# learningmatter-mit/surface-sampling

Measured on AMD Instinct MI355X. Metric: MC energy-evaluations/sec (SrTiO3(001) ~250-atom slabs, 3-model PaiNN ensemble E+F incl. neighbor list), higher is better.
Workload: dtype f32 via fp16x2-split MFMA (3 products), fp32 accumulate; neighbor decisions f64; 1 GPU; SrTiO3(001) PaiNN x3, 256 batched independent chains per GPU (BASELINE configs[3]), 248-272 atoms/chain; chains_per_gpu=256, atoms_per_gpu=66503, edges_per_gpu=2747786, slots_per_gpu=2836316, models=3, streams_per_gpu=2, parallelism=one GPU, no collective

## Files before the change

surface-sampling_amd/csrc/api_painn.hip:

```cpp
#include <cmath>

#include "vssr_internal.h"

namespace vssr {

static void transpose(const float *src, int rows, int cols, float *dst) {
    for (int r = 0; r < rows; ++r)
        for (int c = 0; c < cols; ++c) dst[(size_t)c * rows + r] = src[(size_t)r * cols + c];
}

static int upload_weights(vssr_handle *h, const vssr_painn_config *cfg) {
    const int M = cfg->n_models, L = cfg->num_conv, R = cfg->n_rbf, H = cfg->readout_hidden, NE = cfg->n_embed;
    const size_t per_layer = (size_t)F * F + F + (size_t)F3 * F + F3 + (size_t)F3 * R + F3 + 2 * (size_t)F * F +
                             (size_t)F * 2 * F + F + (size_t)F3 * F + F3;
    const size_t blob_len = (size_t)NE * F + L * per_layer + (size_t)H * F + H + H + 1;
    if (cfg->weights_len != blob_len)
        return set_err(h, VSSR_E_BADARG, "weights_len %llu does not match the layout (%zu floats)",
                       (unsigned long long)cfg->weights_len, blob_len);
    const size_t t_per_layer = (size_t)F * F + (size_t)F * F3 + 2 * (size_t)F * F + (size_t)2 * F * F + (size_t)F * F3;
    const size_t img_len = blob_len + L * t_per_layer + (size_t)F * H;
    std::vector<float> img(img_len * M);
    std::vector<ModelW> table(M);
    if (h->weights.ensure(img.size() * sizeof(float)))
        return set_err(h, VSSR_E_NOMEM, "weights: out of device memory");
// ... 107 lines not shown
            const float *b2 = hb + o; o += F3;
            const float *Wd = hb + o; o += (size_t)F3 * R;
            const float *bd = hb + o;
            l0_build_tables(hb, W1, b1, W2, b2, Wd, bd, NE, A.data() + per_model * m, At.data() + per_model * m);
        }
        const size_t pk = l0_packed_dwords(NE);
        std::vector<unsigned> A16(pk * M), At16(pk * M);
        for (int m = 0; m < M; ++m) l0_pack_tables(A.data() + per_model * m, NE, A16.data() + pk * m, At16.data() + pk * m);
        if (h->d_l0A.ensure(A16.size() * sizeof(unsigned)) || h->d_l0At.ensure(At16.size() * sizeof(unsigned)))
            return set_err(h, VSSR_E_NOMEM, "layer-0 tables");
        VSSR_HIP(h, hipMemcpy(h->d_l0A.p, A16.data(), A16.size() * sizeof(unsigned), hipMemcpyHostToDevice));
        VSSR_HIP(h, hipMemcpy(h->d_l0At.p, At16.data(), At16.size() * sizeof(unsigned), hipMemcpyHostToDevice));
    }
    if (h->model_table.ensure(sizeof(ModelW) * M)) return set_err(h, VSSR_E_NOMEM, "model table");
    VSSR_HIP(h, hipMemcpy(h->model_table.p, table.data(), sizeof(ModelW) * M, hipMemcpyHostToDevice));
    return VSSR_OK;
}

static void read_env_knobs(vssr_handle *h) {
    if (const char *e = getenv("VSSR_PAINN_PATH")) h->painn_general = h->painn_general || strcmp(e, "general") == 0;
    if (const char *e = getenv("VSSR_EDGE_IMPL")) h->edge_impl = (strcmp(e, "gather") == 0) ? 0 : 1;
    if (const char *e = getenv("VSSR_L0_FACTORISE")) h->l0_enabled = atoi(e);
    if (h->painn_general) h->l0_enabled = 0;
    if (const char *e = getenv("VSSR_UPD_SAVE")) h->upd_save = atoi(e);
    if (const char *e = getenv("VSSR_DEBUG_KEEP")) h->debug_keep = atoi(e);
    if (const char *e = getenv("VSSR_EDGE_FS16_MAX")) h->fs16_max_atoms = atoi(e);
    if (const char *e = getenv("VSSR_EDGE_FS8_MAX")) h->fs8_max_atoms = atoi(e);
    if (const char *e = getenv("VSSR_EDGE_BWD_MPASS")) h->bwd_multi_pass = atoi(e);
    if (const char *e = getenv("VSSR_EDGE_SUB_CHUNK")) { const int c = atoi(e); if (c >= 8) { h->sub_chunk_fwd = c; h->sub_chunk_bwd = c; } }
    if (const char *e = getenv("VSSR_EDGE_FWD_2PASS")) { const int w = atoi(e); h->fwd_two_pass = (w == 8 || w == 16) ? w : w ? 16 : 0; }
    if (const char *e = getenv("VSSR_EDGE_FWD_GRID")) h->edge_fwd_grid = max(atoi(e), 0);
}

}

using namespace vssr;

extern "C" {

int vssr_create(const vssr_painn_config *cfg, vssr_handle **out) {
    if (!cfg || !out) return set_err(nullptr, VSSR_E_BADARG, "null argument");
    *out = nullptr;
    if (cfg->struct_size != sizeof(vssr_painn_config))
        return set_err(nullptr, VSSR_E_BADARG, "vssr_painn_config size mismatch (%u vs %zu)", cfg->struct_size,
                       sizeof(vssr_painn_config));
    if (cfg->feat_dim < 16 || cfg->feat_dim > 256 || cfg->feat_dim % 16 != 0 || cfg->n_rbf < 1 || cfg->n_rbf > 32)
// ... 39 lines not shown
```

surface-sampling_amd/csrc/painn.hip:

```cpp
#include "vssr_internal.h"

namespace vssr {

constexpr int T = NODE_TILE;
constexpr int RB = 21;
constexpr int ECHUNK = 16;
constexpr float PI_F = 3.14159265358979323846f;

__device__ inline float sigmoidf_(float x) { return 1.f / (1.f + expf(-x)); }
__device__ inline float swishf_(float x) { return x * sigmoidf_(x); }
__device__ inline float dswishf_(float x) {
    float sg = sigmoidf_(x);
    return sg * fmaf(x, 1.f - sg, 1.f);
}

__global__ void __launch_bounds__(128) k_embed(int N, const int *__restrict__ Z, const ModelW *__restrict__ MW,
                                               float *__restrict__ s0, float *__restrict__ v0) {
    int i = blockIdx.x, m = blockIdx.y, f = threadIdx.x;
    const ModelW &W = MW[m];
    size_t a = (size_t)m * N + i;
    s0[a * F + f] = W.embed[(size_t)Z[i] * F + f];
    v0[(a * 3 + 0) * F + f] = 0.f;
    v0[(a * 3 + 1) * F + f] = 0.f;
    v0[(a * 3 + 2) * F + f] = 0.f;
// ... 556 lines not shown
        for (int c = 0; c < EDGE_MFMA_BCLASSES; o += h->n_bclass[c], ++c) bcls_list[c] = h->d_class_list.as<int>() + o;
    }
    const int n_gather = h->n_class[EDGE_CLASS_GATHER];
    const bool keep = h->upd_save && (want & VSSR_WANT_FORCES) && readout_mfma_supported(H);
    auto save_of = [&](int l) -> void * { return keep ? (char *)h->d_upd_save.p + update_save_bytes(N, M) * (size_t)l : nullptr; };
    h->l0_used = l0_fact;
    const bool fuse_last = readout_mfma_supported(H) && (want & VSSR_WANT_FORCES) && !keep;
    auto update_fwd = [&](int l) {
        const bool last = l + 1 == L;
        if (last && fuse_last && !h->debug_keep) return;
        P.begin(KC_UPDATE_FWD, st);
        launch_update_fwd_mfma(st, N, M, l, av, MW, sv.s_msg[l], sv.v_msg[l], sv.s_in[l + 1],
                               (!last || h->debug_keep) ? sv.v_in[l + 1] : nullptr, !last ? sv.phi[l + 1] : nullptr, save_of(l));
        P.end(st);
    };

    if (!l0_fact) {
        P.begin(KC_EMBED, st);
        hipLaunchKernelGGL(k_embed, g_atom, blk, 0, st, N, Z, MW, sv.s_in[0], sv.v_in[0]);
        P.end(st);
    }
    for (int l = 0; l < L; ++l) {
        if (l == 0 && l0_fact) {
            P.begin(KC_L0_FWD, st);
            rc = l0_run_forward(h, G, sv.s_msg[0], sv.v_msg[0]);
            if (rc) return rc;
            P.end(st);
            update_fwd(l);
            continue;
        }
        if (l == 0) {
            P.begin(KC_MSG_MLP, st);
            launch_msg_mlp_mfma(st, N, M, l, av, MW, sv.s_in[l], sv.phi[l]);
            P.end(st);
        }
        P.begin(KC_EDGE_FWD, st);
        if (l == 0)
            hipLaunchKernelGGL(k_edge_fwd<true>, g_atom, blk, 0, st, N, l, MW, G, counters, h->cutoff, h->excl_vol,
                               h->excl_sigma, h->excl_power, sv.s_in[l], sv.v_in[l], sv.phi[l], sv.s_msg[l],
                               sv.v_msg[l], -1);
        else {
            for (int cls = 0; cls < EDGE_MFMA_CLASSES; ++cls)
                launch_edge_fwd_mfma(st, cls, N, cls_list[cls], h->n_class[cls], M, l, h->max_class_atoms[cls], MW, G, counters,
                                     (int)(h->slot_cap - 1), sv.s_in[l], sv.v_in[l], sv.phi[l], sv.s_msg[l], sv.v_msg[l],
                                     (cls == EDGE_CLASS_FS4 && h->fwd_two_pass) ? h->d_bundle_sub.as<int4>() : (const int4 *)nullptr,
                                     h->fwd_two_pass, h->sub_chunk_fwd ? h->sub_chunk_fwd : sub_chunk_max(h->fwd_two_pass), h->edge_fwd_grid);
            if (n_gather)
                hipLaunchKernelGGL(k_edge_fwd<false>, g_atom, blk, 0, st, N, l, MW, G, counters, h->cutoff, h->excl_vol,
                                   h->excl_sigma, h->excl_power, sv.s_in[l], sv.v_in[l], sv.phi[l], sv.s_msg[l],
                                   sv.v_msg[l], (int)EDGE_BCLASS_GATHER);
        }
// ... 103 lines not shown
```

surface-sampling_amd/csrc/painn_l0.hip:

```cpp
#include "mfma16.h"

namespace vssr {

constexpr int KP = 24;
constexpr int TBLK = 4 * KP;

template <int NZ>
__global__ void __launch_bounds__(96)
k_l0_accum(GraphView G, const int *__restrict__ counters, float *__restrict__ T) {
    constexpr int nz = NZ;
    if (counters[2] || !G.act.atom(blockIdx.x)) return;
    const int i = blockIdx.x, comp = threadIdx.x / KP, kap = threadIdx.x % KP;
    float acc[NZ];
#pragma unroll
    for (int z = 0; z < NZ; ++z) acc[z] = 0.f;
    auto erec_c = [&](int idx) -> float4 {
#if defined(__HIP_DEVICE_COMPILE__)
        typedef const f32x4 __attribute__((address_space(4))) *cp;
        const f32x4 v = reinterpret_cast<cp>(reinterpret_cast<uintptr_t>(G.erec))[idx];
        return make_float4(v.x, v.y, v.z, v.w);
#else
        return G.erec[idx];
#endif
    };
    auto zslot_c = [&](int word) -> unsigned {
#if defined(__HIP_DEVICE_COMPILE__)
        typedef const unsigned __attribute__((address_space(4))) *cp;
// ... 6 lines not shown
    for (int e = e_begin; e < e_end; e += 4) {
        float4 er[4];
        float r[4];
        int zi[4];
        const unsigned zw = zslot_c(e >> 2);
#pragma unroll
        for (int u = 0; u < 4; ++u) {
            er[u] = erec_c(e + u);
            r[u] = G.rho[(size_t)(e + u) * KP + kap];
            zi[u] = (zw >> (8 * u)) & 255;
        }
#pragma unroll
        for (int u = 0; u < 4; ++u) {
            const float uu = comp == 0 ? 1.f : comp == 1 ? er[u].x : comp == 2 ? er[u].y : er[u].z;
            const float val = r[u] * uu;
#pragma unroll
            for (int z = 0; z < NZ; ++z) acc[z] += (z == zi[u]) ? val : 0.f;
        }
    }
#pragma unroll
    for (int z = 0; z < NZ; ++z) T[((size_t)i * nz + z) * TBLK + comp * KP + kap] = acc[z];
}

constexpr int L0_TILE_U4 = 1024;

__global__ void __launch_bounds__(NTHREADS)
k_l0_fwd16(int N, int M, int nz, ActiveView av, const int *__restrict__ counters, const int *__restrict__ Z,
           const int *__restrict__ zlist, const ModelW *__restrict__ MW, const uint4 *__restrict__ A16, int n_embed,
           const float *__restrict__ T, float *__restrict__ s_msg, float *__restrict__ v_msg) {
    extern __shared__ __attribute__((aligned(16))) _Float16 ldsh[];
    if (counters[2]) return;
    const int K = 32 * nz, a0 = blockIdx.x * TA;
    if (!av.tile(min(a0, N - 1), min(a0 + TA - 1, N - 1))) return;
    const Planes Ts = make_planes(ldsh, TA, K), Tv = make_planes(ldsh + plane_halves(TA, K), 3 * TA, K);
    const LaneGeo L;
    SatTrack sat;
    const int lane = threadIdx.x & 63, r = lane & 15, g = lane >> 4;
    for (int t = threadIdx.x; t < TA * nz * 4 * 8; t += NTHREADS) {
        const int k4 = t & 7, comp = (t >> 3) & 3, z = (t >> 5) % nz, a = t / (32 * nz);
        float4 val = make_float4(0.f, 0.f, 0.f, 0.f);
        if (4 * k4 < KP)
            val = *reinterpret_cast<const float4 *>(T + ((size_t)min(a0 + a, N - 1) * nz + z) * TBLK + comp * KP + 4 * k4);
        if (comp == 0) store_split4<SAT_ANY>(Ts, a, 32 * z + 4 * k4, val, sat);
        else store_split4<SAT_ANY>(Tv, (comp - 1) * TA + a, 32 * z + 4 * k4, val, sat);
    }
    sat.commit(av, a0, N);
    __syncthreads();
// ... 229 lines not shown
    for (int z = 0; z < n_embed; ++z)
        for (int sec = 0; sec < 2; ++sec) {
            std::fill(fk.begin(), fk.end(), 0.f);
            std::fill(kf.begin(), kf.end(), 0.f);
            for (int kap = 0; kap < KP; ++kap)
                for (int f = 0; f < F; ++f) {
                    const float v = A[(((size_t)z * 2 + sec) * KP + kap) * F + f];
                    fk[(size_t)f * 32 + kap] = v;
                    kf[(size_t)kap * F + f] = v;
                }
            const size_t o = ((size_t)z * 2 + sec) * L0_TILE_U4 * 4;
            pack_mfma_tiles16(fk.data(), F, 32, A16 + o);
            pack_mfma_tiles16(kf.data(), 32, F, At16 + o);
        }
}
size_t l0_packed_dwords(int n_embed) { return (size_t)n_embed * 2 * L0_TILE_U4 * 4; }

int l0_mfma_init(vssr_handle *h) {
    VSSR_HIP(h, hipFuncSetAttribute((const void *)k_l0_fwd16, hipFuncAttributeMaxDynamicSharedMemorySize, 160 * 1024));
    VSSR_HIP(h, hipFuncSetAttribute((const void *)k_l0_q16, hipFuncAttributeMaxDynamicSharedMemorySize, 160 * 1024));
    return VSSR_OK;
}

int l0_run_forward(vssr_handle *h, const GraphView &G, float *s_msg, float *v_msg) {
    const int N = h->n_atoms, M = h->n_models, nz = h->l0_nz;
    hipStream_t st = h->stream;
    if (h->d_l0T.ensure(sizeof(float) * (size_t)N * nz * TBLK) ||
        h->d_l0Q.ensure(sizeof(float) * (size_t)M * N * nz * TBLK))
        return set_err(h, VSSR_E_NOMEM, "layer-0 factorisation buffers: out of device memory");
    if (!h->l0T_by_geom) {
        const int *cnt = h->d_counters.as<int>();
        float *T = h->d_l0T.as<float>();
        switch (nz) {
            case 1: hipLaunchKernelGGL(k_l0_accum<1>, dim3(N), dim3(96), 0, st, G, cnt, T); break;
            case 2: hipLaunchKernelGGL(k_l0_accum<2>, dim3(N), dim3(96), 0, st, G, cnt, T); break;
            case 3: hipLaunchKernelGGL(k_l0_accum<3>, dim3(N), dim3(96), 0, st, G, cnt, T); break;
            case 4: hipLaunchKernelGGL(k_l0_accum<4>, dim3(N), dim3(96), 0, st, G, cnt, T); break;
            case 5: hipLaunchKernelGGL(k_l0_accum<5>, dim3(N), dim3(96), 0, st, G, cnt, T); break;
            case 6: hipLaunchKernelGGL(k_l0_accum<6>, dim3(N), dim3(96), 0, st, G, cnt, T); break;
            case 7: hipLaunchKernelGGL(k_l0_accum<7>, dim3(N), dim3(96), 0, st, G, cnt, T); break;
            default: hipLaunchKernelGGL(k_l0_accum<L0_MAX_SPECIES>, dim3(N), dim3(96), 0, st, G, cnt, T); break;
        }
    }
    const size_t lds_fwd = sizeof(_Float16) * (plane_halves(TA, 32 * nz) + plane_halves(3 * TA, 32 * nz));
    hipLaunchKernelGGL(k_l0_fwd16, dim3((N + TA - 1) / TA), dim3(NTHREADS), lds_fwd, st, N, M, nz, G.act, h->d_counters.as<int>(),
                       h->d_Z.as<int>(), h->d_zlist.as<int>(), h->model_table.as<ModelW>(), h->d_l0A.as<uint4>(), h->n_embed,
                       h->d_l0T.as<float>(), s_msg, v_msg);
    return VSSR_OK;
}

int l0_run_reverse(vssr_handle *h, const GraphView &G, int first_write, int fresh_mfma, const float *sbar_msg, const float *vbar_msg,
                   float4 *gbar) {
    const int N = h->n_atoms, M = h->n_models, nz = h->l0_nz;
    hipStream_t st = h->stream;
    const size_t lds_q = sizeof(_Float16) * (plane_halves(TA, F) + plane_halves(3 * TA, F));
    hipLaunchKernelGGL(k_l0_q16, dim3((N + TA - 1) / TA, M), dim3(NTHREADS), lds_q, st, N, nz, G.act, h->d_counters.as<int>(),
                       h->d_zlist.as<int>(), h->d_l0At.as<uint4>(), h->n_embed, sbar_msg, vbar_msg, h->d_l0Q.as<float>());
    if (sizeof(float) * 4 * M * nz * TBLK > 48 * 1024)
        VSSR_HIP(h, hipFuncSetAttribute((const void *)k_l0_bwd, hipFuncAttributeMaxDynamicSharedMemorySize, 160 * 1024));
    hipLaunchKernelGGL(k_l0_bwd, dim3((N + 3) / 4), dim3(256), sizeof(float) * 4 * M * nz * TBLK, st, N, M, nz, first_write, fresh_mfma,
                       h->excl_vol, h->cutoff, G, h->d_counters.as<int>(), h->d_l0Q.as<float>(), gbar, (long long)h->slot_cap);
    return VSSR_OK;
}

}
```

surface-sampling_amd/csrc/painn_node_mfma.hip:

```cpp
#include "mfma16.h"

#ifdef PHASE_TIMING
__device__ unsigned long long g_phase[64];
#define PH_INIT unsigned long long ph_t = wall_clock64();
#define PH_RESET ph_t = wall_clock64();
#define PH(k) { const unsigned long long ph_n = wall_clock64(); if (threadIdx.x == 0) atomicAdd(&g_phase[k], ph_n - ph_t); ph_t = wall_clock64(); }
extern "C" int vssr_debug_phases(unsigned long long *out, int reset) {
    if (hipMemcpyFromSymbol(out, HIP_SYMBOL(g_phase), sizeof(unsigned long long) * 64) != hipSuccess) return -1;
    if (reset) { unsigned long long z[64] = {}; if (hipMemcpyToSymbol(HIP_SYMBOL(g_phase), z, sizeof(z)) != hipSuccess) return -1; }
    return 0;
}
#else
#define PH_INIT
#define PH_RESET
#define PH(k)
#endif

namespace vssr {

template <int NRT, int NCT>
struct GemmShape {
    static constexpr int NT = NRT * NCT, NACC = NT >= 3 ? 1 : 2;
};
template <int NRT, int NCT, int NPRE>
// ... 395 lines not shown
        return v_msg + ((mN + a) * 3 + x) * F;
    }, sat);
}
template <int RT, class Sat>
__device__ __forceinline__ void load_update_s(_Float16 *ldsh, const float *__restrict__ s_msg, size_t mN, int a0, int N, Sat &sat) {
    constexpr int TA = 16 * RT;
    const Planes hs = make_planes(ldsh + UpdLds<RT>::OFF_HS, TA, 2 * F);
    load_rows_split<TA>(hs, 0, [&](int row) { return s_msg + (mN + min(a0 + row, N - 1)) * F; }, sat);
}

constexpr int CF_XS = plane_halves(3 * TA, F);
constexpr int CF_LDS_HALVES = CF_XS + plane_halves(TA, F);
static_assert(2 * plane_halves(TA, F) <= CF_XS, "|Vv| and swish planes overlay the v tile");
static_assert(4 * TA * FT * sizeof(float) <= CF_LDS_HALVES * sizeof(_Float16), "output tile overlays the planes");
#ifndef UPD_SAVE_LATE
#define UPD_SAVE_LATE 1
#endif
constexpr int UPD_SAVE_UV = 0, UPD_SAVE_H3 = 12, UPD_SAVE_GATE = 14, UPD_SAVE_REGS = 18;
__device__ __forceinline__ f32x4 &save_slot(f32x4 *save, int m, int k) {
    return save[(((size_t)m * gridDim.x + blockIdx.x) * UPD_SAVE_REGS + k) * NTHREADS + threadIdx.x];
}
size_t update_save_bytes(int N, int M) { return sizeof(f32x4) * (size_t)M * ((N + TA - 1) / TA) * UPD_SAVE_REGS * NTHREADS; }

template <int TAIL>
__global__ void __launch_bounds__(NTHREADS) __attribute__((amdgpu_waves_per_eu(2, 2)))
k_update_fwd_mfma(int N, int l, ActiveView av, const ModelW *__restrict__ MW, const float *__restrict__ s_msg,
                  const float *__restrict__ v_msg, float *__restrict__ s_out, float *__restrict__ v_out,
                  float *__restrict__ phi_next, f32x4 *__restrict__ save) {
    extern __shared__ __attribute__((aligned(16))) _Float16 ldsh[];
    constexpr bool NOV = TAIL == 2;
    const int m = blockIdx.y, a0 = blockIdx.x * TA;
    if (!av.tile(min(a0, N - 1), min(a0 + TA - 1, N - 1))) return;
    const LaneGeo L;
    SatTrack sat;
    const LayerW &W = MW[m].layer[l];
    const size_t mN = (size_t)m * N;
    const Planes vt = make_planes(ldsh, 3 * TA, F), xs = make_planes(ldsh + CF_XS, TA, F);
    const Planes nr = make_planes(ldsh, TA, F), as_ = make_planes(ldsh + plane_halves(TA, F), TA, F);
    constexpr int PF = 1;
    float4 keep_v[3 * TA * (F / 4) / NTHREADS], keep_s[TA * (F / 4) / NTHREADS];
    PH_INIT
    const uint4 *wUV[2] = {WTILE(U, L.w, F), WTILE(V, L.w, F)};
    const uint4 *wW3a[1] = {WTILE(W3, L.w, 2 * F)};
    const uint4 *wW3b[1] = {WTILE(W3, L.w, 2 * F) + (F / 32) * 2 * 64};
    const uint4 *wW4[3] = {WTILE(W4, L.w, F), WTILE(W4, NW + L.w, F), WTILE(W4, 2 * NW + L.w, F)};
    WPre<6, 2, 1> pUV;
    WPre<2, 1, 1> pW3a;
    rows_request<3 * TA>([&](int row) {
        int x = row / TA, a = min(a0 + (row % TA), N - 1);
        return v_msg + ((mN + a) * 3 + x) * F;
    }, keep_v);
    rows_request<TA>([&](int row) { return s_msg + (mN + min(a0 + row, N - 1)) * F; }, keep_s);
    __builtin_amdgcn_sched_barrier(0);
    gemm16_preload(wUV, pUV);
    gemm16_preload(wW3a, pW3a);
    rows_store_split<3 * TA>(vt, 0, keep_v, sat);
    rows_store_split<TA>(xs, 0, keep_s, sat);
    __syncthreads();
    PH(0)
    f32x4 uv[6][2];
    zero_acc(uv);
    gemm16<F, 6, 2, PF, 1>(vt, wUV, uv, &pUV);
    PH(1)
    f32x4 h3[2][1];
    zero_acc(h3);
    gemm16<F, 2, 1, PF, 1>(xs, wW3a, h3, &pW3a);
    WPre<2, 1, 2> pW3b;
    gemm16_preload(wW3b, pW3b);
    PH(2)
    __syncthreads();
    PH(3)
    f32x4 inner[2];
#pragma unroll
    for (int t = 0; t < 2; ++t) {
        f32x4 nv;
#pragma unroll
        for (int i = 0; i < 4; ++i) {
            float n2 = 0.f, in = 0.f;
#pragma unroll
            for (int x = 0; x < 3; ++x) {
// ... 65 lines not shown
        for (int j = 0; j < 6; ++j)
#pragma unroll
            for (int c = 0; c < 2; ++c) save_slot(save, m, UPD_SAVE_UV + 2 * j + c) = uv[j][c];
#pragma unroll
        for (int t = 0; t < 2; ++t) {
            save_slot(save, m, UPD_SAVE_H3 + t) = h3[t][0];
#pragma unroll
            for (int c = 0; c < 2; ++c) save_slot(save, m, UPD_SAVE_GATE + 2 * t + c) = gate[t][c];
        }
    };
#if UPD_SAVE_LATE == 0
    save_all();
#endif
    PH(7)
    __syncthreads();
    PH(8)
    float *T = reinterpret_cast<float *>(ldsh);
#pragma unroll
    for (int t = 0; t < 2; ++t) {
        const int row = L.row(t);
        f32x4 ds;
#pragma unroll
        for (int i = 0; i < 4; ++i) ds[i] = fmaf(gate[t][1][i], inner[t][i], gate[t][2][i]);
        *reinterpret_cast<f32x4 *>(T + row * FT + L.col0) = ds;
        if constexpr (!NOV) {
#pragma unroll
            for (int x = 0; x < 3; ++x) *reinterpret_cast<f32x4 *>(T + (TA * (1 + x) + row) * FT + L.col0) = gate[t][0] * uv[2 * x + t][0];
        }
    }
    __syncthreads();
    auto gofs = [&](int row, int col) -> size_t {
        const int q = row / TA, a = min(a0 + row % TA, N - 1);
        return q == 0 ? (mN + a) * F + col : ((mN + a) * 3 + (q - 1)) * F + col;
    };
    PH(9)
    const Planes xo = make_planes(ldsh + CF_LDS_HALVES, TA, F);
    auto put = [&](int row, int col, const float4 &d, const float4 &r) {
        const float4 o = make_float4(r.x + d.x, r.y + d.y, r.z + d.z, r.w + d.w);
        if (TAIL == 1 && row < TA) store_split4<SAT_COOP>(xo, row, col, o, sat);
        if (a0 + row % TA >= N) return;
        if (row >= TA && !v_out) return;
        *reinterpret_cast<float4 *>((row < TA ? s_out : v_out) + gofs(row, col)) = o;
    };
    {
        constexpr int NS = TA * (F / 4) / NTHREADS, NV = 3 * TA * (F / 4) / NTHREADS;
#pragma unroll
        for (int it = 0; it < (NOV ? NS : NS + NV); ++it) {
            const int idx = threadIdx.x + it * NTHREADS, row = idx >> 5, c4 = idx & 31;
            put(row, 4 * c4, *reinterpret_cast<const float4 *>(T + row * FT + 4 * c4), it < NS ? keep_s[it < NS ? it : 0] : keep_v[it < NS ? 0 : it - NS]);
        }
    }
    PH(10)
    if constexpr (TAIL == 1) {
        const LayerW &Wn = MW[m].layer[l + 1];
        const Planes hn = make_planes(ldsh, TA, F);
        __syncthreads();
        WPre<2, 3, 1> pW2n;
        {
            f32x4 acc[2][1];
            zero_acc(acc);
            const f32x4 b = gload4f(Wn.b1 + L.col0);
            __builtin_amdgcn_sched_barrier(0);
            gemm16<F, 2, 1, 1, 2>(xo, wW1n, acc, &pW1n);
            gemm16_preload(wW2n, pW2n);
#pragma unroll
            for (int t = 0; t < 2; ++t) {
                f32x4 hv = acc[t][0] + b;
#pragma unroll
                for (int i = 0; i < 4; ++i) hv[i] = swish(hv[i]);
                store_split4(hn, L.row(t), L.col0, hv, sat);
            }
        }
        __syncthreads();
        f32x4 acc[2][3];
        zero_acc(acc);
        f32x4 b2[3];
#pragma unroll
        for (int c = 0; c < 3; ++c) b2[c] = gload4f(Wn.b2 + c * F + L.col0);
        __builtin_amdgcn_sched_barrier(0);
        gemm16<F, 2, 3, 1, 1>(hn, wW2n, acc, &pW2n);
#pragma unroll
        for (int c = 0; c < 3; ++c) {
            const f32x4 b = b2[c];
#pragma unroll
            for (int t = 0; t < 2; ++t) {
                const int a = a0 + L.row(t);
                if (a < N) *reinterpret_cast<f32x4 *>(phi_next + (mN + a) * F3 + c * F + L.col0) = acc[t][c] + b;
            }
        }
        PH(11)
    }
#if UPD_SAVE_LATE
    save_all();
#endif
    sat.commit(av, a0, N);
}

constexpr int RH = 64;
template <int RT, bool WANT_SBAR, class Sat>
__device__ __forceinline__ void readout_head(const ModelW &W, const Planes &xs, const Planes &hp, float *red, const LaneGeo &L,
                                             int a0, int N, size_t mN, const float *__restrict__ e_excl,
                                             float *__restrict__ e_atom, f32x4 (&sb)[RT], Sat &sat) {
    constexpr int NCW = RH / 16;
    constexpr int TA = 16 * RT;
    const int lane = threadIdx.x & 63;
    if (L.w < NCW) {
        f32x4 acc[RT][1];
        zero_acc(acc);
        const uint4 *wp[1] = {W.qW5 + (size_t)L.w * 4 * F};
        const f32x4 b = gload4f(W.b5 + L.col0), w6 = gload4f(W.w6 + L.col0);
        __builtin_amdgcn_sched_barrier(0);
        gemm16<F, RT, 1>(xs, wp, acc);
#pragma unroll
        for (int t = 0; t < RT; ++t) {
            const f32x4 hval = acc[t][0] + b;
            f32x4 hb;
            float es = 0.f;
#pragma unroll
// ... 374 lines not shown
        case 1: return sizeof(_Float16) * (plane_halves(TA, F) + plane_halves(TA, F3));
        case 4: return sizeof(_Float16) * (plane_halves(TA, F) + plane_halves(TA, RH)) + sizeof(float) * (RH / 16) * TA;
        case 6: return 96 * 1024;
        default: return sizeof(_Float16) * UpdLds<2>::HALVES + sizeof(float) * 3 * TA * FT;
    }
}
static_assert(sizeof(_Float16) * plane_halves(16, RH) + sizeof(float) * (RH / 16) * 16 <= sizeof(float) * 3 * 16 * FT,
              "readout scratch fits the vbar region");

static_assert(sizeof(_Float16) * (CF_LDS_HALVES + plane_halves(TA, F)) <= 96 * 1024, "update fwd LDS request");

bool readout_mfma_supported(int hidden) { return hidden == RH; }

int node_mfma_init(vssr_handle *h) {
    VSSR_HIP(h, hipFuncSetAttribute((const void *)k_msg_mlp_mfma<2, 0>, hipFuncAttributeMaxDynamicSharedMemorySize, 96 * 1024));
    VSSR_HIP(h, hipFuncSetAttribute((const void *)k_msg_mlp_bwd_mfma, hipFuncAttributeMaxDynamicSharedMemorySize,
                                    (int)node_mfma_lds_bytes(1)));
    VSSR_HIP(h, hipFuncSetAttribute((const void *)k_update_fwd_mfma<0>, hipFuncAttributeMaxDynamicSharedMemorySize,
                                    (int)node_mfma_lds_bytes(6)));
    VSSR_HIP(h, hipFuncSetAttribute((const void *)k_update_fwd_mfma<1>, hipFuncAttributeMaxDynamicSharedMemorySize,
                                    (int)node_mfma_lds_bytes(6)));
    VSSR_HIP(h, hipFuncSetAttribute((const void *)k_update_fwd_mfma<2>, hipFuncAttributeMaxDynamicSharedMemorySize,
                                    (int)node_mfma_lds_bytes(6)));
#define SET_UPD(MODE)                                                                                                     \
    VSSR_HIP(h, hipFuncSetAttribute((const void *)k_update_bwd_mfma<MODE, 2>, hipFuncAttributeMaxDynamicSharedMemorySize, \
                                    (int)node_mfma_lds_bytes(3)));
    SET_UPD(0) SET_UPD(2) SET_UPD(3)
#undef SET_UPD
    VSSR_HIP(h, hipFuncSetAttribute((const void *)k_update_bwd_mfma<1, 2, true>, hipFuncAttributeMaxDynamicSharedMemorySize,
                                    (int)node_mfma_lds_bytes(3)));
    VSSR_HIP(h, hipFuncSetAttribute((const void *)k_update_bwd_mfma<2, 2, true>, hipFuncAttributeMaxDynamicSharedMemorySize,
                                    (int)node_mfma_lds_bytes(3)));
    VSSR_HIP(h, hipFuncSetAttribute((const void *)k_readout_mfma, hipFuncAttributeMaxDynamicSharedMemorySize,
                                    (int)node_mfma_lds_bytes(4)));
    return VSSR_OK;
}

void launch_msg_mlp_mfma(hipStream_t st, int N, int M, int l, const ActiveView &av, const ModelW *MW, const float *s_in,
                         float *phi) {
    hipLaunchKernelGGL((k_msg_mlp_mfma<2, 0>), dim3((N + TA - 1) / TA, M), dim3(NTHREADS), node_mfma_lds_bytes(0), st, N, l, av, MW,
                       s_in, phi);
}
void launch_msg_mlp_bwd_mfma(hipStream_t st, int N, int M, int l, const ActiveView &av, const ModelW *MW, const float *s_in,
                             const float *phibar, const float *sbar_msg, float *sbar_in) {
    hipLaunchKernelGGL(k_msg_mlp_bwd_mfma, dim3((N + TA - 1) / TA, M), dim3(NTHREADS), node_mfma_lds_bytes(1), st, N, l, av, MW,
                       s_in, phibar, sbar_msg, sbar_in);
}
void launch_update_fwd_mfma(hipStream_t st, int N, int M, int l, const ActiveView &av, const ModelW *MW, const float *s_msg,
                            const float *v_msg, float *s_out, float *v_out, float *phi_next, void *save) {
    f32x4 *sv = reinterpret_cast<f32x4 *>(save);
    if (phi_next)
        hipLaunchKernelGGL(k_update_fwd_mfma<1>, dim3((N + TA - 1) / TA, M), dim3(NTHREADS), node_mfma_lds_bytes(6), st, N, l,
                           av, MW, s_msg, v_msg, s_out, v_out, phi_next, sv);
    else if (!v_out && !sv)
        hipLaunchKernelGGL(k_update_fwd_mfma<2>, dim3((N + TA - 1) / TA, M), dim3(NTHREADS), node_mfma_lds_bytes(6), st, N, l,
                           av, MW, s_msg, v_msg, s_out, v_out, phi_next, sv);
    else
        hipLaunchKernelGGL(k_update_fwd_mfma<0>, dim3((N + TA - 1) / TA, M), dim3(NTHREADS), node_mfma_lds_bytes(6), st, N, l,
                           av, MW, s_msg, v_msg, s_out, v_out, phi_next, sv);
}
void launch_readout_mfma(hipStream_t st, int N, int M, const ActiveView &av, const ModelW *MW, const float *s,
                         const float *e_excl, float *e_atom) {
    hipLaunchKernelGGL(k_readout_mfma, dim3((N + TA - 1) / TA, M), dim3(NTHREADS), node_mfma_lds_bytes(4), st, N, av, MW, s,
                       e_excl, e_atom);
}
void launch_update_bwd_mfma(hipStream_t st, int N, int M, int l, int mode, int vbar_is_zero, const ActiveView &av, const ModelW *MW,
                            const float *s_msg, const float *v_msg, const float *sbar_src, const float *vbar,
                            const float *s_next, const float *phibar, const float *e_excl, float *e_atom,
                            float *sbar_msg, float *vbar_msg, float *s_last, const void *save) {
    const f32x4 *sv = reinterpret_cast<const f32x4 *>(save);
    if (mode == 1 || mode == 3) vbar_is_zero = 1;
#if defined(UPD_BWD_RT) && UPD_BWD_RT == 1
    if (!sv && mode == 2) {
        const dim3 grid1((N + 15) / 16, M), blk1(NTHREADS);
        const size_t lds1 = sizeof(_Float16) * UpdLds<1>::HALVES + sizeof(float) * 3 * 16 * FT;
        static bool once = [] {
            (void)hipFuncSetAttribute((const void *)k_update_bwd_mfma<2, 1, false>, hipFuncAttributeMaxDynamicSharedMemorySize, 80 * 1024);
            return true;
        }();
        (void)once;
        hipLaunchKernelGGL((k_update_bwd_mfma<2, 1, false>), grid1, blk1, lds1, st, N, l, vbar_is_zero, av, MW, s_msg, v_msg, sbar_src,
                           vbar, s_next, phibar, e_excl, e_atom, sbar_msg, vbar_msg, s_last, sv);
// ... 17 lines not shown
```

surface-sampling_amd/csrc/vssr_internal.h:

```cpp
#pragma once

#include <hip/hip_runtime.h>

#include <cstdint>
#include <cstdio>
#include <cstdlib>
#include <cstring>
#include <initializer_list>
#include <memory>
#include <string>
#include <type_traits>
#include <utility>
#include <vector>

#include "../../include/vssr_eval.h"

namespace vssr {

constexpr int F = 128;
constexpr int F3 = 3 * F;
constexpr int MAX_LAYERS = 4;
constexpr int MAX_MODELS = 8;
constexpr int RB_MAX = 24;
constexpr int NODE_TILE = 8;
// ... 340 lines not shown
    int cm_cap_per_atom = 0;
    int cg_driver = 0;
    int cg_last_driver = 0;
    bool cap_tight = false;
    vssr::DevBuf d_md_vel;
    vssr::DevBuf d_md_aux;
    bool md_vel_valid = false;
    int md_driver = 0;
    int md_last_driver = 0;
    vssr::DevBuf d_vib;
    vssr::DevBuf d_neb;
    vssr::DevBuf d_dimer;
    vssr::DevBuf d_npt;
    vssr::DevBuf d_cellrelax;
    uint32_t last_want = 0;
    int64_t slot_cap = 0;
    vssr::PinnedInts h_counters;

    vssr::DevBuf d_state;
    vssr::StateView sv;
    vssr::DevBuf d_gbar;
    vssr::DevBuf d_upd_save;
    vssr::DevBuf d_gpart;
    int debug_keep = 0;
    int upd_save = 0;
    vssr::DevBuf d_energy, d_energy_std, d_energy_models, d_forces, d_forces_std, d_e_atoms;
    vssr::DevBuf d_energy64;
    vssr::DevBuf d_pot_e, d_pot_ea, d_pot_f;
    vssr::DevBuf d_sat, d_sat_out;
    std::vector<unsigned> h_sat;
    bool h_sat_valid = false;
    vssr::DevBuf d_stress;

    int gmm_K = 0, gmm_D = 0, gmm_Dp = 0;
    double gmm_log2pi = 0.0;
    vssr::DevBuf d_gmm_P;
    vssr::DevBuf d_gmm_c;
    vssr::DevBuf d_gmm_kc;
    vssr::DevBuf d_gmm_mask;
    vssr::DevBuf d_gmm_x, d_gmm_lp, d_gmm_nll, d_gmm_sys, d_gmm_start;
    std::unique_ptr<vssr::GmmFit> fit;
    std::unique_ptr<vssr::Cluster> clu;
};

namespace vssr {

// ... 104 lines not shown
int chain_min_cg(vssr_handle *h, const vssr_cg_params *cp, const uint8_t *fixed_host, uint32_t want);
int node_mfma_init(vssr_handle *h);
void launch_msg_mlp_mfma(hipStream_t st, int N, int M, int l, const ActiveView &av, const ModelW *MW, const float *s_in,
                         float *phi);
void launch_msg_mlp_bwd_mfma(hipStream_t st, int N, int M, int l, const ActiveView &av, const ModelW *MW, const float *s_in,
                             const float *phibar, const float *sbar_msg, float *sbar_in);
void launch_update_fwd_mfma(hipStream_t st, int N, int M, int l, const ActiveView &av, const ModelW *MW, const float *s_msg,
                            const float *v_msg, float *s_out, float *v_out, float *phi_next, void *save);
size_t update_save_bytes(int N, int M);
bool readout_mfma_supported(int hidden);
void launch_readout_mfma(hipStream_t st, int N, int M, const ActiveView &av, const ModelW *MW, const float *s, const float *e_excl,
                         float *e_atom);
void launch_update_bwd_mfma(hipStream_t st, int N, int M, int l, int mode, int vbar_is_zero, const ActiveView &av, const ModelW *MW,
                            const float *s_msg, const float *v_msg, const float *sbar_src, const float *vbar,
                            const float *s_next, const float *phibar, const float *e_excl, float *e_atom,
                            float *sbar_msg, float *vbar_msg, float *s_last, const void *save);
void pack_mfma_tiles16(const float *Wsrc, int rows, int K, unsigned *dst );
void build_wd16(const float *Wd, const float *bd, unsigned *dst );
void l0_build_tables(const float *blob_embed, const float *W1, const float *b1, const float *W2, const float *b2,
                     const float *Wd, const float *bd, int n_embed, float *A, float *At);
void l0_pack_tables(const float *A, int n_embed, unsigned *A16, unsigned *At16);
size_t l0_packed_dwords(int n_embed);
int l0_mfma_init(vssr_handle *h);
int l0_run_forward(vssr_handle *h, const GraphView &G, float *s_msg, float *v_msg);
int l0_run_reverse(vssr_handle *h, const GraphView &G, int first_write, int fresh_mfma, const float *sbar_msg, const float *vbar_msg,
                   float4 *gbar);
int edge_mfma_init(vssr_handle *h);
enum { EDGE_CLASS_FS16 = 0, EDGE_CLASS_FS16M = 1, EDGE_CLASS_FS8 = 2, EDGE_CLASS_FS4 = 3, EDGE_CLASS_GATHER = 4, EDGE_CLASSES = 5,
       EDGE_MFMA_CLASSES = 4 };
enum { EDGE_BCLASS_FS16 = 0, EDGE_BCLASS_FS8 = 1, EDGE_BCLASS_FS4 = 2, EDGE_BCLASS_FS16P = 3, EDGE_BCLASS_GATHER = 4, EDGE_BCLASSES = 5,
       EDGE_MFMA_BCLASSES = 4 };
__host__ __device__ constexpr int edge_bclass_slices(int c) { return (c == EDGE_BCLASS_FS16 || c == EDGE_BCLASS_FS16P) ? 8 : c == EDGE_BCLASS_FS8 ? 16 : c == EDGE_BCLASS_FS4 ? 32 : 1; }
int edge_bclass_of(int n_atoms);
int edge_class_of(int n_atoms);
constexpr int SUB_MAX_PASSES = 4;
__host__ __device__ constexpr int sub_chunk_max(int width) { return width == 16 ? 400 : 784; }
__host__ __device__ constexpr int sub_chunk_max_bwd() { return 550; }
__host__ __device__ constexpr int sub_passes(int n_atoms, int chunk_max) { return (n_atoms + chunk_max - 1) / chunk_max; }
__host__ __device__ constexpr int sub_chunk(int n_atoms, int chunk_max) { return (n_atoms + sub_passes(n_atoms, chunk_max) - 1) / sub_passes(n_atoms, chunk_max); }
int edge_class_groups(int cls);
void launch_edge_bwd_mfma(hipStream_t st, int cls, int N, const int *list, int n_list, int M, int l, int max_atoms,
                          const ModelW *MW, const GraphView &G, const int *counters, int zero_slot,
                          const float *v_in, const float *phi, const float *sbar_msg, const float *vbar_msg,
                          float *phibar, float *vbar_in, float *gpart, long long slot_cap, int n_groups, int group_off,
                          const int4 *bundle_sub, int sub_chunk);
void launch_edge_fwd_mfma(hipStream_t st, int cls, int N, const int *list, int n_list, int M, int l, int max_atoms, const ModelW *MW,
                          const GraphView &G, const int *counters, int zero_slot, const float *s_in, const float *v_in,
// ... 5 lines not shown
```

Before: 25420 evaluations/s.

## Fuse layer-0 factorised message contraction into the first update kernel

When layer-0 factorisation is active and the number of species is at most four, the separate k_l0_fwd16 contraction kernel is skipped. The first update_fwd kernel now loads the per-atom T tables and packed A16 weights, computes the layer-0 messages with MFMA in its prologue, and adds them directly to the update residual. It still writes s_msg/v_msg for the backward pass. This removes one kernel launch and a global round trip of the message tensors. In exchange the fused kernel needs much more LDS (up to 160 KB), which may lower occupancy.

```diff
diff --git a/surface-sampling_amd/csrc/api_painn.hip b/surface-sampling_amd/csrc/api_painn.hip
--- a/surface-sampling_amd/csrc/api_painn.hip
+++ b/surface-sampling_amd/csrc/api_painn.hip
@@ -153,6 +153,7 @@
     if (const char *e = getenv("VSSR_EDGE_IMPL")) h->edge_impl = (strcmp(e, "gather") == 0) ? 0 : 1;
     if (const char *e = getenv("VSSR_L0_FACTORISE")) h->l0_enabled = atoi(e);
     if (h->painn_general) h->l0_enabled = 0;
+    if (const char *e = getenv("VSSR_L0_FUSE")) h->l0_fuse = atoi(e);
     if (const char *e = getenv("VSSR_UPD_SAVE")) h->upd_save = atoi(e);
     if (const char *e = getenv("VSSR_DEBUG_KEEP")) h->debug_keep = atoi(e);
     if (const char *e = getenv("VSSR_EDGE_FS16_MAX")) h->fs16_max_atoms = atoi(e);
diff --git a/surface-sampling_amd/csrc/painn.hip b/surface-sampling_amd/csrc/painn.hip
--- a/surface-sampling_amd/csrc/painn.hip
+++ b/surface-sampling_amd/csrc/painn.hip
@@ -602,11 +602,19 @@
     }
     for (int l = 0; l < L; ++l) {
         if (l == 0 && l0_fact) {
+            const bool l0_fuse = h->l0_fuse && h->l0T_by_geom && h->l0_nz <= L0_FUSE_MAX_SPECIES && L >= 2;
             P.begin(KC_L0_FWD, st);
-            rc = l0_run_forward(h, G, sv.s_msg[0], sv.v_msg[0]);
+            rc = l0_run_forward(h, G, sv.s_msg[0], sv.v_msg[0], l0_fuse);
             if (rc) return rc;
             P.end(st);
-            update_fwd(l);
+            if (!l0_fuse) {
+                update_fwd(l);
+                continue;
+            }
+            const L0FuseArgs f0{h->d_l0T.as<float>(), h->d_l0A.as<uint4>(), h->d_zlist.as<int>(), Z, counters, h->l0_nz, h->n_embed};
+            P.begin(KC_UPDATE_FWD, st);
+            launch_update_fwd_l0_mfma(st, N, M, av, MW, f0, sv.s_msg[0], sv.v_msg[0], sv.s_in[1], sv.v_in[1], sv.phi[1], save_of(0));
+            P.end(st);
             continue;
         }
         if (l == 0) {
diff --git a/surface-sampling_amd/csrc/painn_l0.hip b/surface-sampling_amd/csrc/painn_l0.hip
--- a/surface-sampling_amd/csrc/painn_l0.hip
+++ b/surface-sampling_amd/csrc/painn_l0.hip
@@ -2,7 +2,7 @@
 
 namespace vssr {
 
-constexpr int KP = 24;
+constexpr int KP = L0_KP;
 constexpr int TBLK = 4 * KP;
 
 template <int NZ>
@@ -55,7 +55,6 @@
     for (int z = 0; z < NZ; ++z) T[((size_t)i * nz + z) * TBLK + comp * KP + kap] = acc[z];
 }
 
-constexpr int L0_TILE_U4 = 1024;
 
 __global__ void __launch_bounds__(NTHREADS)
 k_l0_fwd16(int N, int M, int nz, ActiveView av, const int *__restrict__ counters, const int *__restrict__ Z,
@@ -331,7 +330,7 @@
     return VSSR_OK;
 }
 
-int l0_run_forward(vssr_handle *h, const GraphView &G, float *s_msg, float *v_msg) {
+int l0_run_forward(vssr_handle *h, const GraphView &G, float *s_msg, float *v_msg, bool fused) {
     const int N = h->n_atoms, M = h->n_models, nz = h->l0_nz;
     hipStream_t st = h->stream;
     if (h->d_l0T.ensure(sizeof(float) * (size_t)N * nz * TBLK) ||
@@ -351,6 +350,7 @@
             default: hipLaunchKernelGGL(k_l0_accum<L0_MAX_SPECIES>, dim3(N), dim3(96), 0, st, G, cnt, T); break;
         }
     }
+    if (fused) return VSSR_OK;
     const size_t lds_fwd = sizeof(_Float16) * (plane_halves(TA, 32 * nz) + plane_halves(3 * TA, 32 * nz));
     hipLaunchKernelGGL(k_l0_fwd16, dim3((N + TA - 1) / TA), dim3(NTHREADS), lds_fwd, st, N, M, nz, G.act, h->d_counters.as<int>(),
                        h->d_Z.as<int>(), h->d_zlist.as<int>(), h->model_table.as<ModelW>(), h->d_l0A.as<uint4>(), h->n_embed,
diff --git a/surface-sampling_amd/csrc/painn_node_mfma.hip b/surface-sampling_amd/csrc/painn_node_mfma.hip
--- a/surface-sampling_amd/csrc/painn_node_mfma.hip
+++ b/surface-sampling_amd/csrc/painn_node_mfma.hip
@@ -441,14 +441,17 @@
 }
 size_t update_save_bytes(int N, int M) { return sizeof(f32x4) * (size_t)M * ((N + TA - 1) / TA) * UPD_SAVE_REGS * NTHREADS; }
 
-template <int TAIL>
-__global__ void __launch_bounds__(NTHREADS) __attribute__((amdgpu_waves_per_eu(2, 2)))
-k_update_fwd_mfma(int N, int l, ActiveView av, const ModelW *__restrict__ MW, const float *__restrict__ s_msg,
-                  const float *__restrict__ v_msg, float *__restrict__ s_out, float *__restrict__ v_out,
-                  float *__restrict__ phi_next, f32x4 *__restrict__ save) {
-    extern __shared__ __attribute__((aligned(16))) _Float16 ldsh[];
+struct L0None {};
+template <int TAIL, bool L0F, class L0A>
+__device__ __forceinline__ void
+update_fwd_block(_Float16 *ldsh, int N, int l, const ActiveView &av, const ModelW *__restrict__ MW, const float *__restrict__ s_msg,
+                 const float *__restrict__ v_msg, float *__restrict__ s_out, float *__restrict__ v_out,
+                 float *__restrict__ phi_next, f32x4 *__restrict__ save, const L0A &f0, float *__restrict__ s_msg_w,
+                 float *__restrict__ v_msg_w) {
+    static_assert(!L0F || TAIL == 1, "the fused first block is the TAIL = 1 form");
     constexpr bool NOV = TAIL == 2;
     const int m = blockIdx.y, a0 = blockIdx.x * TA;
+    if constexpr (L0F) { if (f0.counters[2]) return; }
     if (!av.tile(min(a0, N - 1), min(a0 + TA - 1, N - 1))) return;
     const LaneGeo L;
     SatTrack sat;
@@ -457,7 +460,8 @@
     const Planes vt = make_planes(ldsh, 3 * TA, F), xs = make_planes(ldsh + CF_XS, TA, F);
     const Planes nr = make_planes(ldsh, TA, F), as_ = make_planes(ldsh + plane_halves(TA, F), TA, F);
     constexpr int PF = 1;
-    float4 keep_v[3 * TA * (F / 4) / NTHREADS], keep_s[TA * (F / 4) / NTHREADS];
+    float4 keep_v[L0F ? 1 : 3 * TA * (F / 4) / NTHREADS], keep_s[L0F ? 1 : TA * (F / 4) / NTHREADS];
+    f32x4 res[L0F ? 8 : 1];
     PH_INIT
     const uint4 *wUV[2] = {WTILE(U, L.w, F), WTILE(V, L.w, F)};
     const uint4 *wW3a[1] = {WTILE(W3, L.w, 2 * F)};
@@ -465,16 +469,97 @@
     const uint4 *wW4[3] = {WTILE(W4, L.w, F), WTILE(W4, NW + L.w, F), WTILE(W4, 2 * NW + L.w, F)};
     WPre<6, 2, 1> pUV;
     WPre<2, 1, 1> pW3a;
-    rows_request<3 * TA>([&](int row) {
-        int x = row / TA, a = min(a0 + (row % TA), N - 1);
-        return v_msg + ((mN + a) * 3 + x) * F;
-    }, keep_v);
-    rows_request<TA>([&](int row) { return s_msg + (mN + min(a0 + row, N - 1)) * F; }, keep_s);
-    __builtin_amdgcn_sched_barrier(0);
-    gemm16_preload(wUV, pUV);
-    gemm16_preload(wW3a, pW3a);
-    rows_store_split<3 * TA>(vt, 0, keep_v, sat);
-    rows_store_split<TA>(xs, 0, keep_s, sat);
+    if constexpr (L0F) {
+        auto front = [&](auto nzc) {
+            constexpr int NZ = decltype(nzc)::value, K = 32 * NZ, NIT = TA * NZ * 32 / NTHREADS;
+            const int lane = threadIdx.x & 63, g = lane >> 4;
+            _Float16 *tb = ldsh + CF_LDS_HALVES;
+            const Planes Ts = make_planes(tb, TA, K), Tv = make_planes(tb + plane_halves(TA, K), 3 * TA, K);
+            float4 val[NIT];
+#pragma unroll
+            for (int it = 0; it < NIT; ++it) {
+                const int t = threadIdx.x + it * NTHREADS, k4 = t & 7, comp = (t >> 3) & 3, z = (t >> 5) % NZ, a = t / (32 * NZ);
+                val[it] = make_float4(0.f, 0.f, 0.f, 0.f);
+                if (4 * k4 < L0_KP)
+                    val[it] = *reinterpret_cast<const float4 *>(f0.T + ((size_t)min(a0 + a, N - 1) * NZ + z) * (4 * L0_KP) + comp * L0_KP + 4 * k4);
+            }
+            int zz[2];
+#pragma unroll
+            for (int t = 0; t < 2; ++t) zz[t] = f0.Z[min(a0 + L.row(t), N - 1)];
+            u32x4 bw[NZ][2][2];
+#pragma unroll
+            for (int q = 0; q < NZ; ++q) {
+                const uint4 *wb = f0.A16 + (((size_t)m * f0.n_embed + f0.zlist[q]) * 2) * L0_TILE_U4 + (size_t)L.w * 128 + lane;
+#pragma unroll
+                for (int sec = 0; sec < 2; ++sec)
+#pragma unroll
+                    for (int pc = 0; pc < 2; ++pc) bw[q][sec][pc] = gload4u(wb + sec * L0_TILE_U4 + pc * 64);
+            }
+            __builtin_amdgcn_sched_barrier(0);
+            {
+                SatTrack satT;
+#pragma unroll
+                for (int it = 0; it < NIT; ++it) {
+                    const int t = threadIdx.x + it * NTHREADS, k4 = t & 7, comp = (t >> 3) & 3, z = (t >> 5) % NZ, a = t / (32 * NZ);
+                    if (comp == 0) store_split4<SAT_ANY>(Ts, a, 32 * z + 4 * k4, val[it], satT);
+                    else store_split4<SAT_ANY>(Tv, (comp - 1) * TA + a, 32 * z + 4 * k4, val[it], satT);
+                }
+                satT.commit(av, a0, N);
+            }
+            f32x4 emb[2];
+#pragma unroll
+            for (int t = 0; t < 2; ++t) emb[t] = gload4f(MW[m].embed + (size_t)zz[t] * F + L.col0);
+            __syncthreads();
+#pragma unroll
+            for (int t = 0; t < 8; ++t) res[t] = (f32x4){0.f, 0.f, 0.f, 0.f};
+#pragma unroll
+            for (int q = 0; q < NZ; ++q) {
+                u32x4 a[8][2];
+#pragma unroll
+                for (int t = 0; t < 8; ++t) {
+                    const Planes &P = t < 2 ? Ts : Tv;
+                    const int row = (t < 2 ? 16 * t : 16 * (t - 2)) + L.r;
+                    a[t][0] = *reinterpret_cast<const u32x4 *>(P.h + row * P.ld + 32 * q + 8 * g);
+                    a[t][1] = *reinterpret_cast<const u32x4 *>(P.l + row * P.ld + 32 * q + 8 * g);
+                }
+                __builtin_amdgcn_sched_barrier(0);
+#pragma unroll
+                for (int k = 0; k < 3; ++k)
+#pragma unroll
+                    for (int t = 0; t < 8; ++t) {
+                        res[t] = mfma16(bw[q][t < 2 ? 0 : 1][k == 0 ? 1 : 0], a[t][k == 1 ? 1 : 0], res[t]);
+                        __builtin_amdgcn_sched_barrier(0);
+                    }
+            }
+#pragma unroll
+            for (int t = 0; t < 2; ++t) res[t] = emb[t] + res[t];
+        };
+        switch (f0.nz) {
+            case 1: front(std::integral_constant<int, 1>()); break;
+            case 2: front(std::integral_constant<int, 2>()); break;
+            case 3: front(std::integral_constant<int, 3>()); break;
+            default: front(std::integral_constant<int, 4>()); break;
+        }
+        gemm16_preload(wUV, pUV);
+        gemm16_preload(wW3a, pW3a);
+#pragma unroll
+        for (int t = 0; t < 2; ++t) {
+            store_split4<SAT_ACC>(xs, L.row(t), L.col0, res[t], sat);
+#pragma unroll
+            for (int x = 0; x < 3; ++x) store_split4<SAT_ACC>(vt, x * TA + L.row(t), L.col0, res[2 + 2 * x + t], sat);
+        }
+    } else {
+        rows_request<3 * TA>([&](int row) {
+            int x = row / TA, a = min(a0 + (row % TA), N - 1);
+            return v_msg + ((mN + a) * 3 + x) * F;
+        }, keep_v);
+        rows_request<TA>([&](int row) { return s_msg + (mN + min(a0 + row, N - 1)) * F; }, keep_s);
+        __builtin_amdgcn_sched_barrier(0);
+        gemm16_preload(wUV, pUV);
+        gemm16_preload(wW3a, pW3a);
+        rows_store_split<3 * TA>(vt, 0, keep_v, sat);
+        rows_store_split<TA>(xs, 0, keep_s, sat);
+    }
     __syncthreads();
     PH(0)
     f32x4 uv[6][2];
@@ -586,10 +671,15 @@
         f32x4 ds;
 #pragma unroll
         for (int i = 0; i < 4; ++i) ds[i] = fmaf(gate[t][1][i], inner[t][i], gate[t][2][i]);
+        if constexpr (L0F) ds = res[t] + ds;
         *reinterpret_cast<f32x4 *>(T + row * FT + L.col0) = ds;
         if constexpr (!NOV) {
 #pragma unroll
-            for (int x = 0; x < 3; ++x) *reinterpret_cast<f32x4 *>(T + (TA * (1 + x) + row) * FT + L.col0) = gate[t][0] * uv[2 * x + t][0];
+            for (int x = 0; x < 3; ++x) {
+                f32x4 dv = gate[t][0] * uv[2 * x + t][0];
+                if constexpr (L0F) dv = res[2 + 2 * x + t] + dv;
+                *reinterpret_cast<f32x4 *>(T + (TA * (1 + x) + row) * FT + L.col0) = dv;
+            }
         }
     }
     __syncthreads();
@@ -600,7 +690,7 @@
     PH(9)
     const Planes xo = make_planes(ldsh + CF_LDS_HALVES, TA, F);
     auto put = [&](int row, int col, const float4 &d, const float4 &r) {
-        const float4 o = make_float4(r.x + d.x, r.y + d.y, r.z + d.z, r.w + d.w);
+        const float4 o = L0F ? d : make_float4(r.x + d.x, r.y + d.y, r.z + d.z, r.w + d.w);
         if (TAIL == 1 && row < TA) store_split4<SAT_COOP>(xo, row, col, o, sat);
         if (a0 + row % TA >= N) return;
         if (row >= TA && !v_out) return;
@@ -611,7 +701,20 @@
 #pragma unroll
         for (int it = 0; it < (NOV ? NS : NS + NV); ++it) {
             const int idx = threadIdx.x + it * NTHREADS, row = idx >> 5, c4 = idx & 31;
-            put(row, 4 * c4, *reinterpret_cast<const float4 *>(T + row * FT + 4 * c4), it < NS ? keep_s[it < NS ? it : 0] : keep_v[it < NS ? 0 : it - NS]);
+            float4 r = make_float4(0.f, 0.f, 0.f, 0.f);
+            if constexpr (!L0F) r = it < NS ? keep_s[it < NS ? it : 0] : keep_v[it < NS ? 0 : it - NS];
+            put(row, 4 * c4, *reinterpret_cast<const float4 *>(T + row * FT + 4 * c4), r);
+        }
+    }
+    if constexpr (L0F) {
+#pragma unroll
+        for (int t = 0; t < 2; ++t) {
+            const int a_ = a0 + L.row(t);
+            if (a_ < N) {
+                *reinterpret_cast<f32x4 *>(s_msg_w + (mN + a_) * F + L.col0) = res[t];
+#pragma unroll
+                for (int x = 0; x < 3; ++x) *reinterpret_cast<f32x4 *>(v_msg_w + ((mN + a_) * 3 + x) * F + L.col0) = res[2 + 2 * x + t];
+            }
         }
     }
     PH(10)
@@ -658,6 +761,23 @@
     save_all();
 #endif
     sat.commit(av, a0, N);
+}
+
+template <int TAIL>
+__global__ void __launch_bounds__(NTHREADS) __attribute__((amdgpu_waves_per_eu(2, 2)))
+k_update_fwd_mfma(int N, int l, ActiveView av, const ModelW *__restrict__ MW, const float *__restrict__ s_msg,
+                  const float *__restrict__ v_msg, float *__restrict__ s_out, float *__restrict__ v_out,
+                  float *__restrict__ phi_next, f32x4 *__restrict__ save) {
+    extern __shared__ __attribute__((aligned(16))) _Float16 ldsh[];
+    update_fwd_block<TAIL, false>(ldsh, N, l, av, MW, s_msg, v_msg, s_out, v_out, phi_next, save, L0None(), nullptr, nullptr);
+}
+
+__global__ void __launch_bounds__(NTHREADS) __attribute__((amdgpu_waves_per_eu(2, 2)))
+k_update_fwd_l0_mfma(int N, ActiveView av, const ModelW *__restrict__ MW, L0FuseArgs f0, float *__restrict__ s_msg,
+                     float *__restrict__ v_msg, float *__restrict__ s_out, float *__restrict__ v_out,
+                     float *__restrict__ phi_next, f32x4 *__restrict__ save) {
+    extern __shared__ __attribute__((aligned(16))) _Float16 ldsh[];
+    update_fwd_block<1, true>(ldsh, N, 0, av, MW, nullptr, nullptr, s_out, v_out, phi_next, save, f0, s_msg, v_msg);
 }
 
 constexpr int RH = 64;
@@ -1078,6 +1198,7 @@
                                     (int)node_mfma_lds_bytes(6)));
     VSSR_HIP(h, hipFuncSetAttribute((const void *)k_update_fwd_mfma<2>, hipFuncAttributeMaxDynamicSharedMemorySize,
                                     (int)node_mfma_lds_bytes(6)));
+    VSSR_HIP(h, hipFuncSetAttribute((const void *)k_update_fwd_l0_mfma, hipFuncAttributeMaxDynamicSharedMemorySize, 160 * 1024));
 #define SET_UPD(MODE)                                                                                                     \
     VSSR_HIP(h, hipFuncSetAttribute((const void *)k_update_bwd_mfma<MODE, 2>, hipFuncAttributeMaxDynamicSharedMemorySize, \
                                     (int)node_mfma_lds_bytes(3)));
@@ -1114,6 +1235,14 @@
     else
         hipLaunchKernelGGL(k_update_fwd_mfma<0>, dim3((N + TA - 1) / TA, M), dim3(NTHREADS), node_mfma_lds_bytes(6), st, N, l,
                            av, MW, s_msg, v_msg, s_out, v_out, phi_next, sv);
+}
+void launch_update_fwd_l0_mfma(hipStream_t st, int N, int M, const ActiveView &av, const ModelW *MW, const L0FuseArgs &f0,
+                               float *s_msg, float *v_msg, float *s_out, float *v_out, float *phi_next, void *save) {
+    const int K = 32 * f0.nz;
+    const size_t lds = std::max(node_mfma_lds_bytes(6),
+                                sizeof(_Float16) * (CF_LDS_HALVES + plane_halves(TA, K) + plane_halves(3 * TA, K)));
+    hipLaunchKernelGGL(k_update_fwd_l0_mfma, dim3((N + TA - 1) / TA, M), dim3(NTHREADS), lds, st, N, av, MW, f0, s_msg, v_msg,
+                       s_out, v_out, phi_next, reinterpret_cast<f32x4 *>(save));
 }
 void launch_readout_mfma(hipStream_t st, int N, int M, const ActiveView &av, const ModelW *MW, const float *s,
                          const float *e_excl, float *e_atom) {
diff --git a/surface-sampling_amd/csrc/vssr_internal.h b/surface-sampling_amd/csrc/vssr_internal.h
--- a/surface-sampling_amd/csrc/vssr_internal.h
+++ b/surface-sampling_amd/csrc/vssr_internal.h
@@ -386,6 +386,7 @@
     vssr::DevBuf d_gbar;
     vssr::DevBuf d_upd_save;
     vssr::DevBuf d_gpart;
+    int l0_fuse = 1;
     int debug_keep = 0;
     int upd_save = 0;
     vssr::DevBuf d_energy, d_energy_std, d_energy_models, d_forces, d_forces_std, d_e_atoms;
@@ -536,7 +537,18 @@
 void l0_pack_tables(const float *A, int n_embed, unsigned *A16, unsigned *At16);
 size_t l0_packed_dwords(int n_embed);
 int l0_mfma_init(vssr_handle *h);
-int l0_run_forward(vssr_handle *h, const GraphView &G, float *s_msg, float *v_msg);
+int l0_run_forward(vssr_handle *h, const GraphView &G, float *s_msg, float *v_msg, bool fused);
+constexpr int L0_KP = 24;
+constexpr int L0_TILE_U4 = 1024;
+constexpr int L0_FUSE_MAX_SPECIES = 4;
+struct L0FuseArgs {
+    const float *T;
+    const uint4 *A16;
+    const int *zlist, *Z, *counters;
+    int nz, n_embed;
+};
+void launch_update_fwd_l0_mfma(hipStream_t st, int N, int M, const ActiveView &av, const ModelW *MW, const L0FuseArgs &f0,
+                               float *s_msg, float *v_msg, float *s_out, float *v_out, float *phi_next, void *save);
 int l0_run_reverse(vssr_handle *h, const GraphView &G, int first_write, int fresh_mfma, const float *sbar_msg, const float *vbar_msg,
                    float4 *gbar);
 int edge_mfma_init(vssr_handle *h);
```

After: 25520 evaluations/s, median of 6. About the same (+0.4%).
